# facebookresearch/SEAL

Measured on NVIDIA H100. Metric: queries/sec at beam=15, 1k queries, 10M-token index; rank-kernel HBM GB/s, higher is better.
Workload: dtype f32

## Files before the change

### include/sealdec.h

```cpp
#ifndef SEALDEC_H
#define SEALDEC_H
#include <stdint.h>
#include "sealfm.h"

#ifdef __cplusplus
extern "C" {
#endif


typedef struct {
    int32_t num_beams;
    int32_t pad_token_id;
    int32_t eos_token_id;
    int32_t stop_at_count;
    int32_t always_allow_eos;
    int32_t forced_bos_token_id;
    int32_t n_force_decoding_from;
    const int64_t* force_decoding_from;
    int32_t shift;
} sealdec_processor_cfg_t;

int sealdec_apply_index_mask_d(const sealfm_t* fm, sealfm_stream_t stream,
                               const sealdec_processor_cfg_t* cfg,
                               const int64_t* input_ids_d, int64_t R, int64_t t,
// ... 118 lines not shown
                           int64_t Q, int64_t S, const int64_t* dec_ids, const int32_t* row_query,
                           int64_t N, int64_t T, float temperature, float* out_logprob,
                           int64_t out_full_pos, float* out_full);

int sealdec_debug_step_logits(sealbart_t* model, const int64_t* input_ids, const int64_t* attention_mask,
                              int64_t Q, int64_t S, int32_t num_beams, const int64_t* decoder_input_ids,
                              int64_t t, float* out_logits);
int sealdec_debug_step_logits_ex(sealbart_t* model, const int64_t* input_ids, const int64_t* attention_mask,
                                 int64_t Q, int64_t S, int32_t num_beams, const int64_t* decoder_input_ids,
                                 int64_t t, const int32_t* ancestry, int64_t src_tokens_hint, float* out_logits);
int sealdec_debug_gemm(int mode, int64_t M, int32_t N, int32_t K, const float* A, const float* W,
                       const float* bias, float* C, int32_t gelu, int32_t iters, double* avg_us);
int sealdec_debug_gemm_ex(int mode, int64_t M, int32_t N, int32_t K, const float* A, const float* W,
                          const float* bias, float* C, int32_t gelu, int32_t iters, double* avg_us, int32_t band,
                          int32_t store);
int sealdec_debug_head(int64_t M, int32_t N, int32_t K, const float* A, const float* W, const float* bias,
                       const uint32_t* mask, int32_t eos, int32_t pad, float* C, float* stats, int32_t* fused);
int sealdec_debug_head_ex(int mode, int64_t M, int32_t N, int32_t K, const float* A, const float* W, const float* bias,
                          const uint32_t* mask, int32_t eos, int32_t pad, float* C, float* stats, int32_t* fused);
int sealdec_debug_select_step(const sealfm_t* fm, const sealdec_params_t* p, const sealdec_groups_t* groups, int64_t Q,
                              int32_t V, int32_t cur_len, int32_t logits_shared, int32_t logits_ignored,
                              const float* logits, const float* head_stats, const uint32_t* masks,
                              const uint32_t* occurring_mask, const float* beam_scores, const int32_t* tokens,
                              const int32_t* ancestry, const uint64_t* lo, const uint64_t* hi, const uint64_t* pw,
                              float* row_max, float* row_logsum, uint8_t* row_rule, float* cand_val, int32_t* cand_idx,
                              int32_t* cand_cnt, int32_t* lists, float* beam_scores_out, int32_t* tokens_out,
                              int32_t* ancestry_out, uint64_t* lo_out, uint64_t* hi_out, uint64_t* pw_out,
                              float* rec_score, int32_t* rec_len, int32_t* rec_tokens, uint8_t* rec_valid,
                              uint64_t* rec_lo, uint64_t* rec_hi, int32_t* error_flag);
int sealdec_debug_target_logprob(int64_t R, int32_t V, int64_t ld, const float* logits, const int64_t* targets,
                                 int64_t tgt_stride, float temperature, float* out, int64_t out_stride, float* full,
                                 int64_t full_ld);
typedef struct {
    int32_t kind, arch, d, heads;
    int64_t Q, S;
    int32_t B, pos, T, compact;
    const float* qkv; const float* q; const float* ckv;
    const float* kc; const float* vc; const int32_t* anc;
    const int32_t* src_mask; const int32_t* src_off;
    int64_t G; const int32_t* grp_query; const int32_t* grp_start;
    const float* rel_bias; int32_t num_buckets, max_distance;
    const float* split_part; int32_t split_ks; float split_unscale; const float* split_bias;
    int32_t out_split;
} sealdec_attn_case_t;
int sealdec_debug_attention(const sealdec_attn_case_t* c, float* out, void* split1, void* split2, void* split3,
                            int32_t* overflow, float* kc_out, float* vc_out, uint32_t* path);
int sealdec_debug_topk_threshold(int64_t R, int32_t V, int64_t ld, const float* logits, int32_t top_k, float* out_thr,
                                 float* out_max, float* out_logsum);
int sealdec_debug_topk_threshold_cluster(int64_t R, int32_t V, int64_t ld, const float* logits, int32_t top_k,
                                         float* out_thr, float* out_max, float* out_logsum);
int sealdec_debug_topk_rows(int64_t R, int32_t V, int32_t num_beams, int32_t per_row, int32_t iters, double* avg_us);
int sealdec_debug_gemm_trace(int enable, int64_t out20[20]);
int sealdec_debug_gemm_units(int64_t* out, int32_t n);
int64_t sealdec_last_launch_count(const sealbart_t* model);
int sealdec_profile_gemm(sealbart_t* model, int enable, double* total_us, int64_t* launches, double* flops);
int sealdec_last_phase_us(const sealbart_t* model, double out5[5]);

#ifdef __cplusplus
}
#endif
#endif
```

### seal_b200/_lib.py

```python
import ctypes as C
import os

_HERE = os.path.dirname(os.path.abspath(__file__))
LIB_PATH = os.path.join(_HERE, "libsealb200.so")

u64 = C.c_uint64
u32 = C.c_uint32
i32 = C.c_int
vp = C.c_void_p
cp = C.c_char_p


class SealB200Error(RuntimeError):
    def __init__(self, code, msg):
        super().__init__(f"[sealb200 {code}] {msg}")
        self.code = code


def _load():
    if not os.path.exists(LIB_PATH):
        raise ImportError(
            f"{LIB_PATH} not found: build it with `python -c 'import __graft_entry__ as g; g.build()'` "
            "or `make -C seal_b200/csrc`. seal_b200 has no CPU fallback.")
    return C.CDLL(LIB_PATH)
# ... 97 lines not shown
                ("B", C.c_int32), ("pos", C.c_int32), ("T", C.c_int32), ("compact", C.c_int32),
                ("qkv", vp), ("q", vp), ("ckv", vp), ("kc", vp), ("vc", vp), ("anc", vp),
                ("src_mask", vp), ("src_off", vp),
                ("G", C.c_int64), ("grp_query", vp), ("grp_start", vp),
                ("rel_bias", vp), ("num_buckets", C.c_int32), ("max_distance", C.c_int32),
                ("split_part", vp), ("split_ks", C.c_int32), ("split_unscale", C.c_float), ("split_bias", vp),
                ("out_split", C.c_int32)]


_DEC_SIGS = {
    "sealdec_apply_index_mask_d": (i32, [vp, vp, C.POINTER(ProcessorCfg), vp, C.c_int64, C.c_int64, vp, vp, vp,
                                         C.c_int64, C.c_int64]),
    "sealbart_create": (i32, [C.POINTER(BartConfig), i32, C.POINTER(vp)]),
    "sealbart_create_ex": (i32, [C.POINTER(BartConfig), C.POINTER(BartVariant), i32, C.POINTER(vp)]),
    "sealbart_free": (None, [vp]),
    "sealt5_create": (i32, [C.POINTER(T5Config), i32, C.POINTER(vp)]),
    "sealt5_relative_buckets": (i32, [C.c_int32, C.c_int32, C.c_int32, C.c_int32, vp]),
    "sealbart_set_tensor": (i32, [vp, cp, vp, u64]),
    "sealbart_finalize": (i32, [vp]),
    "sealbart_device_bytes": (u64, [vp]),
    "sealdec_hyps_per_query": (C.c_int64, [C.POINTER(DecParams)]),
    "sealdec_generate": (i32, [vp, vp, vp, C.POINTER(DecParams), vp, vp, C.c_int64, C.c_int64, vp, vp, vp, vp, vp, vp]),
    "sealdec_generate_d": (i32, [vp, vp, vp, C.POINTER(DecParams), vp, vp, C.c_int64, C.c_int64, vp, vp, vp, vp, vp,
                                 vp, vp, vp]),
    "sealdec_generate_dx": (i32, [vp, vp, vp, C.POINTER(DecParams), vp, vp, C.c_int64, C.c_int64, vp, vp, vp, vp, vp,
                                  vp, vp, vp, C.c_int64]),
    "sealdec_generate_ex": (i32, [vp, vp, vp, C.POINTER(DecParams), vp, vp, C.c_int64, C.c_int64, vp, vp, vp, vp, vp, vp,
                                  C.POINTER(GroupParams)]),
    "sealdec_generate_dx_ex": (i32, [vp, vp, vp, C.POINTER(DecParams), vp, vp, C.c_int64, C.c_int64, vp, vp, vp, vp, vp,
                                     vp, vp, vp, C.c_int64, C.POINTER(GroupParams)]),
    "sealbart_set_option": (i32, [vp, cp, C.c_int64]),
    "sealbart_get_stat": (C.c_int64, [vp, cp]),
    "sealdec_teacher_forced": (i32, [vp, vp, vp, C.c_int64, C.c_int64, vp, vp, C.c_int64, C.c_int64, C.c_float, vp,
                                     C.c_int64, vp]),
    "sealdec_debug_step_logits": (i32, [vp, vp, vp, C.c_int64, C.c_int64, C.c_int32, vp, C.c_int64, vp]),
    "sealdec_debug_step_logits_ex": (i32, [vp, vp, vp, C.c_int64, C.c_int64, C.c_int32, vp, C.c_int64, vp, C.c_int64,
                                           vp]),
    "sealdec_debug_gemm": (i32, [i32, C.c_int64, C.c_int32, C.c_int32, vp, vp, vp, vp, C.c_int32, C.c_int32,
                                 C.POINTER(C.c_double)]),
    "sealdec_debug_gemm_ex": (i32, [i32, C.c_int64, C.c_int32, C.c_int32, vp, vp, vp, vp, C.c_int32, C.c_int32,
                                    C.POINTER(C.c_double), C.c_int32, C.c_int32]),
    "sealdec_debug_head": (i32, [C.c_int64, C.c_int32, C.c_int32, vp, vp, vp, vp, C.c_int32, C.c_int32, vp, vp, vp]),
    "sealdec_debug_head_ex": (i32, [i32, C.c_int64, C.c_int32, C.c_int32, vp, vp, vp, vp, C.c_int32, C.c_int32, vp, vp, vp]),
    "sealdec_debug_select_step": (i32, [vp, C.POINTER(DecParams), C.POINTER(GroupParams), C.c_int64, C.c_int32, C.c_int32,
                                        C.c_int32, C.c_int32] + [vp] * 30),
    "sealdec_debug_target_logprob": (i32, [C.c_int64, C.c_int32, C.c_int64, vp, vp, C.c_int64, C.c_float, vp, C.c_int64,
                                           vp, C.c_int64]),
    "sealdec_debug_attention": (i32, [C.POINTER(AttnCase), vp, vp, vp, vp, vp, vp, vp, vp]),
    "sealdec_debug_topk_threshold": (i32, [C.c_int64, C.c_int32, C.c_int64, vp, C.c_int32, vp, vp, vp]),
    "sealdec_debug_topk_threshold_cluster": (i32, [C.c_int64, C.c_int32, C.c_int64, vp, C.c_int32, vp, vp, vp]),
    "sealdec_debug_topk_rows":(i32, [C.c_int64, C.c_int32, C.c_int32, C.c_int32, C.c_int32, C.POINTER(C.c_double)]),
    "sealdec_debug_gemm_trace": (i32, [i32, C.POINTER(C.c_int64)]),
    "sealdec_debug_gemm_units": (i32, [C.POINTER(C.c_int64), C.c_int32]),
    "sealev_first_stage": (i32, [C.c_int64, vp, vp, vp, vp, C.c_int64, vp, vp, vp, i32, i32, C.c_double, C.c_double, C.c_int64, vp, vp]),
    "sealev_score_docs": (i32, [C.c_int64, vp, vp, vp, vp, C.c_int64, C.c_int64, vp, vp, vp, C.c_int64, i32, i32, i32, i32,
                                C.c_double, C.c_double, vp, vp, vp, vp, vp, vp, C.c_int64]),
    "sealev_last_error": (C.c_char_p, []),
    "sealev_set_sum_mode": (None, [i32]),
    "sealev_key_scores": (i32, [C.c_int64, vp, vp, vp, vp, C.c_double, C.c_double, C.c_double, C.c_double, i32, vp]),
    "sealev_unigram_topk": (i32, [C.c_int64, C.c_int64, vp, C.c_int64, vp, vp, vp, vp]),
    "sealev_unigram_scores": (i32, [C.c_int64, vp, vp, vp, C.c_double, C.c_double, C.c_double, i32, vp]),
    "sealev_best_unigrams": (i32, [C.c_int64, vp, vp, vp, vp, vp, vp, vp, vp, C.c_int64]),
    "sealev_set_device_budget": (None, [u64]),
    "sealev_batch_first_stage": (i32, [vp, C.c_int64, vp, vp, vp, vp, vp, vp, vp, vp, i32, i32, C.c_double, C.c_double,
                                       C.c_int64, vp, vp, C.c_int64]),
    "sealev_batch_score_docs": (i32, [vp, C.c_int64, vp, vp, vp, vp, vp, vp, vp, vp, vp, vp, vp, vp, C.c_int64, i32, i32,
                                      i32, i32, C.c_double, C.c_double, vp, vp, C.c_int64, vp, vp, vp, vp, vp, vp,
                                      C.c_int64, vp]),
    "sealev_batch_phase_us": (None, [vp]),
    "sealdec_last_launch_count": (C.c_int64, [vp]),
    "sealdec_profile_gemm": (i32, [vp, i32, C.POINTER(C.c_double), C.POINTER(C.c_int64), C.POINTER(C.c_double)]),
    "sealdec_last_phase_us": (i32, [vp, C.POINTER(C.c_double)]),
}


def _bind(sigs):
    for name, (res, args) in sigs.items():
        fn = getattr(lib, name)
        fn.restype = res
        fn.argtypes = args


_bind(_FM_SIGS)
_bind(_DEC_SIGS)


def check(code):
    if code != 0:
        raise SealB200Error(code, lib.sealfm_last_error().decode(errors="replace"))


def fm_symbols():
    return list(_FM_SIGS)
```

### seal_b200/csrc/bart_kernels.cuh

```cuda
#pragma once
#include <cuda_bf16.h>
#include <cuda_fp16.h>
#include <cuda_runtime.h>
#include <cstdint>

#include "decode_types.cuh"
#include "launch.cuh"

namespace sealb200 {

__device__ __forceinline__ float warp_sum(float v) {
#pragma unroll
    for (int o = 16; o > 0; o >>= 1) v += __shfl_xor_sync(0xffffffffu, v, o);
    return v;
}
__device__ __forceinline__ float warp_max(float v) {
#pragma unroll
    for (int o = 16; o > 0; o >>= 1) v = fmaxf(v, __shfl_xor_sync(0xffffffffu, v, o));
    return v;
}

__device__ __forceinline__ void split1(float x, float& h, float& l) {
    h = __uint_as_float(__float_as_uint(x) & 0xFFFFE000u);
    l = x - h;
// ... 334 lines not shown
        if (rd * 4 < n_keys && s < n_keys) {
            const float p = expf(sc[rd] - mloc);
            lsum += p;
            const float4 v0 = vf[rd][0], v1 = vf[rd][1];
            a0.x = fmaf(p, v0.x, a0.x); a0.y = fmaf(p, v0.y, a0.y); a0.z = fmaf(p, v0.z, a0.z); a0.w = fmaf(p, v0.w, a0.w);
            a1.x = fmaf(p, v1.x, a1.x); a1.y = fmaf(p, v1.y, a1.y); a1.z = fmaf(p, v1.z, a1.z); a1.w = fmaf(p, v1.w, a1.w);
        }
    }
#pragma unroll
    for (int o = 8; o <= 16; o <<= 1) {
        lsum += __shfl_xor_sync(0xffffffffu, lsum, o);
        a0.x += __shfl_xor_sync(0xffffffffu, a0.x, o); a0.y += __shfl_xor_sync(0xffffffffu, a0.y, o);
        a0.z += __shfl_xor_sync(0xffffffffu, a0.z, o); a0.w += __shfl_xor_sync(0xffffffffu, a0.w, o);
        a1.x += __shfl_xor_sync(0xffffffffu, a1.x, o); a1.y += __shfl_xor_sync(0xffffffffu, a1.y, o);
        a1.z += __shfl_xor_sync(0xffffffffu, a1.z, o); a1.w += __shfl_xor_sync(0xffffffffu, a1.w, o);
    }
    const float inv = 1.0f / lsum;
    o0 = make_float4(a0.x * inv, a0.y * inv, a0.z * inv, a0.w * inv);
    o1 = make_float4(a1.x * inv, a1.y * inv, a1.z * inv, a1.w * inv);
}

template <int ROUNDS, class SO>
__global__ void __launch_bounds__(512, ROUNDS <= 3 ? 2 : 1) dec_self_attn_kernel(int64_t R, int d, int heads, int cur_pos, int T,
                                                               const float* __restrict__ qkv, float* kc, float* vc,
                                                               const int32_t* __restrict__ anc,
                                                               float* __restrict__ out, SO so, int row_mul, int bcast) {
    const int64_t r = blockIdx.x;
    const int64_t pr = r * row_mul;
    const int lane = threadIdx.x & 31, warp = threadIdx.x >> 5;
    const int g = lane >> 3, i8 = (lane & 7) * 8;
    const int n_keys = cur_pos + 1;
    const int32_t* arow = anc + pr * T;
    for (int h = warp; h < heads; h += blockDim.x >> 5) {
        const int col = h * kHeadDim + i8;
        const float* qp = qkv + r * 3 * d + col;
        float4 o0, o1;
        self_attend_head<ROUNDS>(qp, kc, vc, arow, R, d, col, cur_pos, n_keys, g, o0, o1);
        if (g == 0) {
            const int64_t idx = r * d + col;
            if (out) { *reinterpret_cast<float4*>(out + idx) = o0; *reinterpret_cast<float4*>(out + idx + 4) = o1; }
            store_split4(so, idx, o0); store_split4(so, idx + 4, o1);
            const float* kcur = qp + d; const float* vcur = qp + 2 * d;
            const float4 k0 = __ldg(reinterpret_cast<const float4*>(kcur)), k1 = __ldg(reinterpret_cast<const float4*>(kcur + 4));
            const float4 v0 = __ldg(reinterpret_cast<const float4*>(vcur)), v1 = __ldg(reinterpret_cast<const float4*>(vcur + 4));
            for (int b2 = 0; b2 < bcast; ++b2) {
                float* kd = kc + ((int64_t)cur_pos * R + pr + b2) * d + col; float* vd = vc + ((int64_t)cur_pos * R + pr + b2) * d + col;
                *reinterpret_cast<float4*>(kd) = k0; *reinterpret_cast<float4*>(kd + 4) = k1;
                *reinterpret_cast<float4*>(vd) = v0; *reinterpret_cast<float4*>(vd + 4) = v1;
            }
        }
    }
}

__host__ __device__ inline size_t self_attn_query_smem(int P, int B) { return (size_t)2 * P * B * kHeadDim * 4 + (size_t)2 * P * 32 * 4 + 128 * 4; }

template <class SO>
__global__ void __launch_bounds__(1024) dec_self_attn_query_kernel(int64_t R, int B, int d, int cur_pos, int T,
                                                                  const float* __restrict__ qkv, float* kc, float* vc,
                                                                  const int32_t* __restrict__ anc,
                                                                  float* __restrict__ out, SO so, SplitSrc qsrc) {
    extern __shared__ __align__(16) unsigned char sa_smem[];
    const int P = cur_pos + 1;
    float* Ks = reinterpret_cast<float*>(sa_smem);
    float* Vs = Ks + (size_t)P * B * kHeadDim;
    int32_t* row_of = reinterpret_cast<int32_t*>(Vs + (size_t)P * B * kHeadDim);
    int32_t* slot_of = row_of + P * 32;
    int32_t* ucount = slot_of + P * 32;
    const int64_t qi = blockIdx.x;
    const int col = blockIdx.y * kHeadDim;
    const int64_t r0 = qi * B;
    const int lane = threadIdx.x & 31, warp = threadIdx.x >> 5;
    for (int s = warp; s < P; s += B) {
        const bool act = lane < B;
        const unsigned amask = __ballot_sync(0xffffffffu, act);
        if (act) {
            const int a = (s == cur_pos) ? lane : anc[(r0 + lane) * T + s];
            const unsigned same = __match_any_sync(amask, a);
            const int leader = __ffs(same) - 1;
            const unsigned leaders = __ballot_sync(amask, leader == lane);
            slot_of[s * 32 + lane] = __popc(leaders & ((1u << leader) - 1u));
            if (leader == lane) row_of[s * 32 + __popc(leaders & ((1u << lane) - 1u))] = a;
            if (lane == 0) ucount[s] = __popc(leaders);
        }
    }
    __syncthreads();
    const int per_pos = B * (kHeadDim / 4);
    for (int e = threadIdx.x; e < P * per_pos; e += blockDim.x) {
        const int s = e / per_pos, rem = e - s * per_pos, slot = rem / (kHeadDim / 4), i4 = rem - slot * (kHeadDim / 4);
        if (slot >= ucount[s]) continue;
        const int a = row_of[s * 32 + slot];
        float4 kk, vv;
        if (s == cur_pos) {
            const int64_t qoff = (r0 + a) * 3 * d + col + 4 * i4;
            kk = load_split4(qkv, qsrc, qoff + d, d + col + 4 * i4); vv = load_split4(qkv, qsrc, qoff + 2 * d, 2 * d + col + 4 * i4);
            const int64_t off = ((int64_t)cur_pos * R + r0 + a) * d + col + 4 * i4;
            *reinterpret_cast<float4*>(kc + off) = kk; *reinterpret_cast<float4*>(vc + off) = vv;
        } else {
            const int64_t off = ((int64_t)s * R + a) * d + col + 4 * i4;
            kk = *reinterpret_cast<const float4*>(kc + off); vv = *reinterpret_cast<const float4*>(vc + off);
        }
        *reinterpret_cast<float4*>(Ks + ((size_t)s * B + slot) * kHeadDim + 4 * i4) = kk;
        *reinterpret_cast<float4*>(Vs + ((size_t)s * B + slot) * kHeadDim + 4 * i4) = vv;
    }
    __syncthreads();
    if (warp < B) {
        const int64_t r = r0 + warp;
        const float2 q2 = load_split2(qkv, qsrc, r * 3 * d + col + 2 * lane, col + 2 * lane);
        float m = -INFINITY, l = 0.f, ax = 0.f, ay = 0.f;
        for (int s = 0; s < P; ++s) {
            const int slot = slot_of[s * 32 + warp];
            const float2 k2 = *reinterpret_cast<const float2*>(Ks + ((size_t)s * B + slot) * kHeadDim + 2 * lane);
            const float sc = warp_sum(q2.x * k2.x + q2.y * k2.y) * 0.125f;
            const float mn = fmaxf(m, sc);
            const float corr = (m == -INFINITY) ? 0.f : expf(m - mn);
            const float p = expf(sc - mn);
            const float2 v2 = *reinterpret_cast<const float2*>(Vs + ((size_t)s * B + slot) * kHeadDim + 2 * lane);
            l = l * corr + p;
            ax = fmaf(p, v2.x, ax * corr); ay = fmaf(p, v2.y, ay * corr);
            m = mn;
        }
        store_attn(make_float2(ax / l, ay / l), r * d + col + 2 * lane, out, so);
    }
}

struct AncestryKV {
    const float* kc; const float* vc; const int32_t* arow; const float* kcur; const float* vcur;
    int64_t R; int d; int col; int cur_pos;
    __device__ __forceinline__ bool valid(int) const { return true; }
    __device__ __forceinline__ const float* k(int s) const { return s == cur_pos ? kcur : kc + ((int64_t)s * R + arow[s]) * d + col; }
    __device__ __forceinline__ const float* v(int s) const { return s == cur_pos ? vcur : vc + ((int64_t)s * R + arow[s]) * d + col; }
};

template <class SO>
__global__ void __launch_bounds__(512) dec_self_attn_long_kernel(int64_t R, int d, int heads, int cur_pos, int T,
                                                                 const float* __restrict__ qkv, float* kc, float* vc,
                                                                 const int32_t* __restrict__ anc,
                                                                 float* __restrict__ out, SO so) {
    __shared__ __align__(16) float q_s[16][kHeadDim];
    const int64_t r = blockIdx.x;
    const int lane = threadIdx.x & 31, warp = threadIdx.x >> 5;
    const int32_t* arow = anc + r * T;
    for (int h = warp; h < heads; h += blockDim.x >> 5) {
        const int col = h * kHeadDim;
        const float* qp = qkv + r * 3 * d + col;
        AncestryKV kv{kc, vc, arow, qp + d, qp + 2 * d, R, d, col, cur_pos};
        const float2 o = warp_attend(qp, cur_pos + 1, kv, q_s[warp]);
        store_attn(o, r * d + col + 2 * lane, out, so);
        const float2 k2 = *reinterpret_cast<const float2*>(qp + d + 2 * lane);
        const float2 v2 = *reinterpret_cast<const float2*>(qp + 2 * d + 2 * lane);
        *reinterpret_cast<float2*>(kc + ((int64_t)cur_pos * R + r) * d + col + 2 * lane) = k2;
        *reinterpret_cast<float2*>(vc + ((int64_t)cur_pos * R + r) * d + col + 2 * lane) = v2;
    }
}

struct GroupAddr {
    const float* q; int64_t q_stride;
    const float* k; const float* v; int64_t kv_stride;
    const int32_t* mask;
};

template <int NW, int MAXP, class SO>
__device__ __forceinline__ void grouped_attention(const GroupAddr& g, int rows, int n_keys, int head_off, int64_t out_base,
                                                  int64_t out_stride, float* __restrict__ out, const SO& so) {
    __shared__ float Kt[kHeadDim][33];
    __shared__ __align__(16) float Vs[32][kHeadDim];
    __shared__ __align__(16) float q_s[NW * MAXP][kHeadDim];
    __shared__ int32_t valid_s[32];
    const int lane = threadIdx.x & 31, warp = threadIdx.x >> 5;
    for (int rbase = 0; rbase < rows; rbase += NW * MAXP) {
        float m[MAXP], l[MAXP], ax[MAXP], ay[MAXP];
        bool has[MAXP];
#pragma unroll
        for (int p = 0; p < MAXP; ++p) {
            const int r = rbase + p * NW + warp;
// ... 194 lines not shown
```

### seal_b200/csrc/decode_model.hpp

```cpp
#pragma once
#include "../../include/sealdec.h"
#include "common.cuh"
#include "decode_types.cuh"

#include <cuda.h>
#include <cuda_bf16.h>
#include <cuda_fp16.h>
#include <cuda_runtime.h>

#include <cstdint>
#include <map>
#include <set>
#include <string>
#include <utility>
#include <vector>

#pragma GCC visibility push(hidden)

namespace sealb200 {

struct Lin {
    float* w = nullptr; float* b = nullptr; int out = 0, in = 0;
    float* w_hi = nullptr; float* w_lo = nullptr;
    __half* w_h1 = nullptr; __half* w_h2 = nullptr;
// ... 84 lines not shown
    int graph_policy = -1;
    int last_used_graph = 0;
    bool tf32_ready = false;
    int64_t overflow_fallbacks = 0;
    cudaStream_t stream = nullptr;
    int query_slices = -1;
    cudaStream_t slice_stream = nullptr;
    cudaEvent_t slice_fork = nullptr, slice_join = nullptr;
    Buf a_hi1, a_lo1, splitk1, st_wide1;
    Buf effn2, dffn2;
    ~sealbart() { for (void* p : allocs) cudaFree(p); for (void* p : split_allocs) cudaFree(p); }
};

namespace sealb200 {

enum GemmMode : int { kGemmTf32 = 2, kGemmFp16 = 3, kGemmFp16Cluster = 5, kGemmBf16 = 6 };
inline bool is_3xfp16(int64_t mode) { return mode == kGemmFp16 || mode == kGemmFp16Cluster; }
inline bool head_stats_mode(int mode) { return mode == kGemmFp16 || mode == kGemmBf16; }
inline bool bf16_weights(const sealbart* m) { return m->cfg.gemm_mode == kGemmBf16; }

constexpr int64_t kAddLnRowMax = 2048;

struct Act {
    float* x = nullptr; float* hi = nullptr; float* lo = nullptr;
    __half* h1 = nullptr; __half* h2 = nullptr;
    __nv_bfloat16* b1 = nullptr; __nv_bfloat16* b2 = nullptr; __nv_bfloat16* b3 = nullptr;
};

struct Ctx { sealbart* m; cudaStream_t s; SplitSrc pending{}; HeadEpi head{}; bool head_fused = false; int slice = 0; };

struct Dims {
    int64_t Q, S, R; int B, T, d, f, V, ld, W;
    int64_t G = 0; const int32_t* grp_query = nullptr; const int32_t* grp_start = nullptr;
    int64_t q0 = 0, r0 = 0, Qb = 0, Rb = 0;
};

template <typename Fn> void for_each_lin(sealbart* m, Fn&& fn) {
    for (auto& L : m->enc) { fn(L.qkv); fn(L.o); fn(L.fc1); fn(L.fc2); }
    for (auto& L : m->dec) { fn(L.qkv); fn(L.o); fn(L.cq); fn(L.ckv); fn(L.co); fn(L.fc1); fn(L.fc2); }
    fn(m->head);
}

void make_lin(sealbart* m, Lin& l, int out, int in);
void upload(void* dst, bool bf16, const float* host, uint64_t n, float scale = 1.f);
void check_model(const sealbart* m);
int require_device();
void ensure_workspace(sealbart* m, const Dims& D);
int32_t t5_bucket(int32_t rel, bool bidirectional, int num_buckets, int max_distance);

void gemm(Ctx& cx, int64_t M, int N, int K, const Act& A, int lda, Lin& l, const Act& C, int ldc, int act, int64_t defer_rows = 0);
void derive_lin(sealbart* m, Lin& l, unsigned int* d_max);
void ensure_tf32_splits(sealbart* m);
void check_gemm_mode(int mode);

void encoder_forward(Ctx& cx, const Dims& D, const int64_t* ids_d, const int64_t* mask_d, int64_t src_tokens_hint = -1,
                     int32_t* hint_err = nullptr);
void decoder_step(Ctx& cx, const Dims& D, const int32_t* tokens, int cur_len, const int32_t* anc, bool want_logits,
                  cudaEvent_t ev_layers_done, bool compact = false, const HeadEpi& head = HeadEpi{});

void drop_graphs(sealbart* m);

}

#pragma GCC visibility pop
```

### seal_b200/csrc/forward.cu

```cuda
#include "decode_model.hpp"
#include "bart_kernels.cuh"
#include "preln_kernels.cuh"
#include "t5_kernels.cuh"

#include <cuda_runtime.h>

#include <algorithm>
#include <cmath>
#include <cstdlib>
#include <type_traits>
#include <vector>

namespace {

SplitSrc take_pending(Ctx& cx) {
    const SplitSrc ps = cx.pending;
    cx.pending = SplitSrc{};
    return ps;
}

SplitOut split_of(const Act& a, int* overflow) {
    SplitOut so;
    if (a.hi) { so.a = a.hi; so.b = a.lo; so.kind = 1; }
    else if (a.h1) { so.a = a.h1; so.b = a.h2; so.kind = 2; so.overflow = overflow; }
// ... 68 lines not shown
    int64_t run = part[t];
    for (int64_t q = q0; q < q1; ++q) {
        src_off[q] = (int32_t)run;
        int len = 0;
        for (int s2 = 0; s2 < S; ++s2) len += mask[q * S + s2] != 0;
        run += len;
    }
    if (t == 0) src_off[Q] = (int32_t)info[0];
}

__global__ void prep_enc_packed_kernel(int64_t n, int S, const int64_t* __restrict__ ids, const int32_t* __restrict__ src_off,
                                       int32_t* __restrict__ tok, int32_t* __restrict__ pos) {
    const int64_t i = blockIdx.x * (int64_t)blockDim.x + threadIdx.x;
    if (i >= n) return;
    const int64_t q = i / S; const int s2 = (int)(i % S);
    if (s2 < src_off[q + 1] - src_off[q]) { const int64_t dst = src_off[q] + s2; tok[dst] = (int32_t)ids[i]; pos[dst] = s2; }
}

void t5_rms(Ctx& cx, int64_t rows, int d, const int32_t* tok, int64_t tok_stride, const Act& x, const float* b, const float* w,
            float out_scale) {
    const SplitSrc ps = take_pending(cx);
    const bool wide = d > 4 * 128 * kT5RmsVec;
    with_split(cx.m, x, [&](auto so) {
        using SO = decltype(so);
        launch_k(wide ? t5_rms_row_kernel<kT5RmsVecWide, SO> : t5_rms_row_kernel<kT5RmsVec, SO>, (unsigned)rows, 128, 0, cx.s, rows, d, tok, tok_stride,
                 embed_table<SO>(cx.m), x.x, b, ps, w, cx.m->t5.layer_norm_epsilon, out_scale, so);
    });
    cx.m->launches++;
    cx.m->last_paths |= wide ? kPathT5RmsWide : kPathT5Rms;
}

void t5_ffn(Ctx& cx, int64_t rows, int d, int f, const Act& x, Lin& fc1, Lin& fc2, const Act& ffn, float* ffn2, const Act& tmp) {
    sealbart* m = cx.m;
    if (m->t5.ffn_kind == 1) {
        gemm(cx, rows, 2 * f, d, x, d, fc1, Act{ffn2}, 2 * f, kActNone);
        const int blocks = (int)std::max<int64_t>(1, std::min<int64_t>((rows * (f / 4) + 255) / 256, (int64_t)sm_count() * 8));
        with_split(m, ffn, [&](auto so) { launch_k(t5_gate_kernel<decltype(so)>, (unsigned)blocks, 256, 0, cx.s, rows, f, (const float*)ffn2, so); });
        m->launches++; m->last_paths |= kPathT5Gate;
    } else
        gemm(cx, rows, f, d, x, d, fc1, ffn, f, kActRelu);
    gemm(cx, rows, d, f, ffn, f, fc2, tmp, d, kActNone, INT64_MAX);
}

struct Acts { Act x, qkv, attn, tmp, cq, ffn; float* ffn2 = nullptr; };

struct DecStep : Acts {
    int64_t R = 0, Rc = 0, Tk = 0, ckv_q0 = 0; int row_mul = 1, pos = 0; bool compact = false;
    const int32_t* tokens = nullptr; const int32_t* anc = nullptr; const int32_t* m32 = nullptr; const int32_t* soff_x = nullptr;
};


bool use_self_attn_query(int pos, int B, bool compact, bool ragged) {
    static const bool sa_query = [] { const char* e = std::getenv("SEALB200_SELF_ATTN_QUERY"); return !e || std::atoi(e) != 0; }();
    const size_t saq_smem = self_attn_query_smem(pos + 1, B);
    return sa_query && !compact && !ragged && pos >= 1 && B >= 2 && B <= 32 && pos + 1 <= 128 && saq_smem <= 112 * 1024;
}

bool use_cross_attn_small(int64_t S) { return S <= kXKeys; }

struct SelfAttnArgs {
    int64_t Q, R, Rc; int B, d, heads, pos, T, row_mul;
    const float* qkv; float* kc; float* vc; const int32_t* anc; float* out;
};

template <class SO>
uint32_t launch_bart_self_attn(cudaStream_t s, const SelfAttnArgs& a, bool use_saq, const SO& so, const SplitSrc& qkv_src) {
    const unsigned sa_threads = 32 * std::min(a.heads, 16);
    if (use_saq) {
        static size_t saq_set = 0;
        const size_t saq_smem = self_attn_query_smem(a.pos + 1, a.B);
        if (saq_smem > saq_set) { CUDA_CHECK(cudaFuncSetAttribute(dec_self_attn_query_kernel<SO>, cudaFuncAttributeMaxDynamicSharedMemorySize, 112 * 1024)); saq_set = 112 * 1024; }
        launch_k(dec_self_attn_query_kernel<SO>, dim3((unsigned)a.Q, a.heads), 32 * a.B, saq_smem, s, a.Rc, a.B, a.d, a.pos, a.T, a.qkv, a.kc, a.vc, a.anc,
                 a.out, so, qkv_src);
        return kPathSelfQuery;
    }
    if (a.pos + 1 <= 12) {
        launch_k(dec_self_attn_kernel<3, SO>, (unsigned)a.R, sa_threads, 0, s, a.Rc, a.d, a.heads, a.pos, a.T, a.qkv, a.kc, a.vc, a.anc, a.out, so, a.row_mul, a.row_mul);
        return kPathSelfRounds3;
    }
    if (a.pos + 1 <= 32) {
        launch_k(dec_self_attn_kernel<8, SO>, (unsigned)a.R, sa_threads, 0, s, a.Rc, a.d, a.heads, a.pos, a.T, a.qkv, a.kc, a.vc, a.anc, a.out, so, a.row_mul, a.row_mul);
        return kPathSelfRounds8;
    }
    launch_k(dec_self_attn_long_kernel<SO>, (unsigned)a.R, sa_threads, 0, s, a.Rc, a.d, a.heads, a.pos, a.T, a.qkv, a.kc, a.vc, a.anc, a.out, so);
    return kPathSelfLong;
}

template <class SO>
uint32_t launch_t5_dec_self_attn(cudaStream_t s, const SelfAttnArgs& a, const RelBias& rb, const SO& so) {
    launch_k(t5_dec_self_attn_kernel<SO>, (unsigned)a.R, 32 * std::min(a.heads, 16), 0, s, a.Rc, a.d, a.heads, a.pos, a.T, a.qkv, a.kc, a.vc,
             a.anc, rb, so, a.row_mul, a.row_mul);
    return kPathT5DecAttn;
}

struct CrossAttnArgs {
    int64_t groups; int d, heads, beams, S;
    const float* q; const float* ckv; const int32_t* mask; const int32_t* grp_query; const int32_t* grp_start; float* out;
    const int32_t* src_off;
};

template <class SO>
uint32_t launch_cross_attn(cudaStream_t s, const CrossAttnArgs& a, const SO& so, const SplitSrc& q_src) {
    if (use_cross_attn_small(a.S)) {
        launch_k(cross_attn_small_kernel<SO>, dim3((unsigned)a.groups, a.heads), 128, 0, s, a.groups, a.d, a.heads, a.beams, a.S, a.q,
                 a.ckv, a.mask, a.grp_query, a.grp_start, a.out, so, a.src_off, q_src);
        return kPathCrossSmall;
    }
    launch_k(cross_attn_kernel<SO>, dim3((unsigned)a.groups, a.heads), kGAttnWarps * 32, 0, s, a.groups, a.d, a.heads, a.beams, a.S, a.q,
             a.ckv, a.mask, a.grp_query, a.grp_start, a.out, so, a.src_off);
    return kPathCrossGrouped;
}

template <class SO>
uint32_t launch_enc_self_attn(cudaStream_t s, int64_t Q, int d, int heads, int S, const float* qkv, const int32_t* mask,
                              const RelBias* rb, float* out, const SO& so, const int32_t* src_off) {
    if (rb) {
        launch_k(t5_enc_self_attn_kernel<kGAttnWarps, kGAttnPasses, SO>, dim3((unsigned)Q, heads), kGAttnWarps * 32, 0, s, Q, d, S, qkv, mask, *rb,
                 so, src_off);
        return kPathT5EncAttn;
    }
    launch_k(enc_self_attn_kernel<SO>, dim3((unsigned)Q, heads), kGAttnWarps * 32, 0, s, Q, d, heads, S, qkv, mask, out, so, src_off);
    return 0;
}

void cross_attention(Ctx& cx, const Dims& D, const DecStep& S, int l, int64_t defer_rows) {
    sealbart* m = cx.m;
// ... 347 lines not shown
            else up(d_mask, c->src_mask, (size_t)Q * c->S * 4);
        }
        const size_t cache_bytes = self ? (size_t)c->T * Rc * d * 4 : 0;
        if (self) {
            up(d_kc, c->kc, cache_bytes); up(d_vc, c->vc, cache_bytes); up(d_anc, c->anc, (size_t)Rc * c->T * 4);
            const size_t at_pos = (size_t)c->pos * Rc * d * 4, pos_bytes = (size_t)Rc * d * 4;
            CUDA_CHECK(cudaMemset(d_kc.as<char>() + at_pos, 0xFF, pos_bytes)); CUDA_CHECK(cudaMemset(d_vc.as<char>() + at_pos, 0xFF, pos_bytes));
        }
        if (cross && c->G) { up(d_gq, c->grp_query, (size_t)c->G * 4); up(d_gs, c->grp_start, (size_t)(c->G + 1) * 4); }
        RelBias rb{};
        if (t5_bias) {
            const int off = enc ? kT5MaxSource - 1 : kMaxLen - 1;
            std::vector<int32_t> bkt(enc ? 2 * kT5MaxSource - 1 : kMaxLen);
            for (int i = 0; i < (int)bkt.size(); ++i) bkt[i] = t5_bucket(i - off, enc, c->num_buckets, c->max_distance);
            up(d_bkt, bkt.data(), bkt.size() * 4); up(d_rel, c->rel_bias, (size_t)c->num_buckets * heads * 4);
            rb = RelBias{d_rel.as<float>(), d_bkt.as<int32_t>(), off, heads};
        }
        const size_t out_n = (size_t)rows * d, piece = c->out_split == 1 ? 4 : 2;
        nan(d_out, out_n * 4);
        if (c->out_split) { nan(d_s1, out_n * piece); nan(d_s2, out_n * piece); }
        if (c->out_split == 3) nan(d_s3, out_n * piece);
        d_ovf.ensure(4); CUDA_CHECK(cudaMemset(d_ovf.p, 0, 4));
        SplitSrc src{};
        if (c->split_ks > 1) src = SplitSrc{d_part.as<float>(), c->split_ks, (int64_t)rows * cols, d_pb.as<float>(), c->split_unscale};

        const float* in = d_in.as<float>();
        const int32_t* mask = c->src_off ? nullptr : d_mask.as<int32_t>();
        const int32_t* soff = c->src_off ? d_off.as<int32_t>() : nullptr;
        auto run = [&](auto so) -> uint32_t {
            if (enc) return launch_enc_self_attn(nullptr, Q, d, heads, (int)c->S, in, mask, t5 ? &rb : nullptr, d_out.as<float>(), so, soff);
            if (self) {
                const SelfAttnArgs a{Q, rows, Rc, c->B, d, heads, c->pos, c->T, c->compact ? c->B : 1, in, d_kc.as<float>(), d_vc.as<float>(),
                                     d_anc.as<int32_t>(), d_out.as<float>()};
                return t5 ? launch_t5_dec_self_attn(nullptr, a, rb, so) : launch_bart_self_attn(nullptr, a, use_saq, so, src);
            }
            const CrossAttnArgs a{c->G ? c->G : Q, d, heads, c->compact ? 1 : c->B, (int)c->S, in, d_ckv.as<float>(), mask,
                                  c->G ? d_gq.as<int32_t>() : nullptr, c->G ? d_gs.as<int32_t>() : nullptr, d_out.as<float>(), soff};
            return launch_cross_attn(nullptr, a, so, src);
        };
        uint32_t bit;
        if (c->out_split == 3) bit = run(SplitBf16{d_s1.as<__nv_bfloat16>(), d_s2.as<__nv_bfloat16>(), d_s3.as<__nv_bfloat16>()});
        else bit = run(SplitOut{d_s1.p, d_s2.p, c->out_split, c->out_split == 2 ? d_ovf.as<int>() : nullptr});
        CUDA_CHECK(cudaDeviceSynchronize());
        auto down = [&](void* h, const Buf& b, size_t bytes) { CUDA_CHECK(cudaMemcpy(h, b.p, bytes, cudaMemcpyDeviceToHost)); };
        down(out, d_out, out_n * 4);
        if (c->out_split) { down(split1, d_s1, out_n * piece); down(split2, d_s2, out_n * piece); }
        if (c->out_split == 3) down(split3, d_s3, out_n * piece);
        if (overflow) down(overflow, d_ovf, 4);
        if (self) { down(kc_out, d_kc, cache_bytes); down(vc_out, d_vc, cache_bytes); }
        *path = bit;
    });
}

}
```

### seal_b200/csrc/gemm.cu

```cuda
#include "decode_model.hpp"
#include "wgmma_gemm.cuh"

#include <cuda_runtime.h>

#include <algorithm>
#include <cmath>
#include <cstdlib>
#include <cstring>
#include <iterator>
#include <type_traits>
#include <vector>

namespace {

typedef CUresult (*EncodeTiledFn)(CUtensorMap*, CUtensorMapDataType, cuuint32_t, void*, const cuuint64_t*, const cuuint64_t*,
                                  const cuuint32_t*, const cuuint32_t*, CUtensorMapInterleave, CUtensorMapSwizzle,
                                  CUtensorMapL2promotion, CUtensorMapFloatOOBfill);
EncodeTiledFn encode_tiled() {
    static EncodeTiledFn fn = nullptr;
    if (!fn) {
        void* p = nullptr;
        cudaDriverEntryPointQueryResult q;
        CUDA_CHECK(cudaGetDriverEntryPoint("cuTensorMapEncodeTiled", &p, cudaEnableDefault, &q));
        if (!p || q != cudaDriverEntryPointSuccess) throw ApiError(SEALFM_ECUDA, "cuTensorMapEncodeTiled unavailable");
// ... 206 lines not shown
}

void split_lin_half(sealbart* m, Lin& l, unsigned int* d_max) {
    const uint64_t n = (uint64_t)l.out * l.in;
    CUDA_CHECK(cudaMemset(d_max, 0, 4));
    absmax_kernel<<<sm_count() * 4, 256>>>((int64_t)n, l.w, d_max);
    unsigned int bits = 0; CUDA_CHECK(cudaMemcpy(&bits, d_max, 4, cudaMemcpyDeviceToHost));
    float mx; std::memcpy(&mx, &bits, 4);
    int sexp = 0;
    if (mx > 0.f) { int e; std::frexp(mx, &e); sexp = 14 - e; }
    l.w_unscale = std::ldexp(1.0f, -sexp);
    CUDA_CHECK(cudaMalloc(&l.w_h1, n * 2)); m->split_allocs.push_back(l.w_h1);
    CUDA_CHECK(cudaMalloc(&l.w_h2, n * 2)); m->split_allocs.push_back(l.w_h2);
    m->weight_bytes += 2 * n * 2;
    split_half_kernel<<<sm_count() * 8, 256>>>((int64_t)n, l.w, std::ldexp(1.0f, sexp), l.w_h1, l.w_h2, m->err.as<int>() + 1);
    CUDA_CHECK(cudaGetLastError());
    l.maps_ready = false;
}

}

namespace sealb200 {

void gemm(Ctx& cx, int64_t M, int N, int K, const Act& A, int lda, Lin& l, const Act& C, int ldc, int act, int64_t defer_rows) {
    sealbart* m = cx.m;
    if (!m->profile_gemm || M == 0) { gemm_impl(cx, M, N, K, A, lda, l, C, ldc, act, defer_rows); return; }
    cudaEvent_t a, b;
    CUDA_CHECK(cudaEventCreate(&a)); CUDA_CHECK(cudaEventCreate(&b));
    CUDA_CHECK(cudaEventRecord(a, cx.s));
    gemm_impl(cx, M, N, K, A, lda, l, C, ldc, act, defer_rows);
    CUDA_CHECK(cudaEventRecord(b, cx.s));
    m->gemm_events.emplace_back(a, b);
    m->gemm_flops += 2.0 * (double)M * N * K;
}

void derive_lin(sealbart* m, Lin& l, unsigned int* d_max) {
    if (m->cfg.gemm_mode == kGemmTf32) split_lin_tf32(m, l);
    else if (is_3xfp16(m->cfg.gemm_mode)) split_lin_half(m, l, d_max);
}

void ensure_tf32_splits(sealbart* m) {
    if (m->tf32_ready) return;
    CUDA_CHECK(cudaSetDevice(m->device));
    for_each_lin(m, [&](Lin& l) { split_lin_tf32(m, l); });
    CUDA_CHECK(cudaDeviceSynchronize());
    m->tf32_ready = true;
}

void check_gemm_mode(int mode) {
    if (mode != kGemmTf32 && !is_3xfp16(mode) && mode != kGemmBf16)
        throw ApiError(SEALFM_EINVAL, "gemm_mode must be 3 (3xFP16, one CTA per tile, default), 5 (3xFP16 on 2-CTA clusters), 2 (3xTF32) "
                                      "or 6 (3xBF16, bf16 weights)");
}

}


extern "C" {

int sealdec_debug_gemm_trace(int enable, int64_t out20[20]) {
    return guarded([&] {
        if (out20) {
            CUDA_CHECK(cudaDeviceSynchronize());
            long long h[20];
            CUDA_CHECK(cudaMemcpyFromSymbol(h, g_gemm_trace, sizeof(h)));
            for (int i = 0; i < 20; ++i) out20[i] = h[i];
        }
        const int on = enable ? 1 : 0;
        CUDA_CHECK(cudaMemcpyToSymbol(g_gemm_trace_on, &on, sizeof(int)));
    });
}

int sealdec_debug_gemm_units(int64_t* out, int32_t n) {
    return guarded([&] {
        if (!out || n < 0 || n > 4 * kTraceUnits) throw ApiError(SEALFM_EINVAL, "out is null or n is outside [0, 4 * 256]");
#ifndef SEAL_GEMM_UNIT_TRACE
        throw ApiError(SEALFM_EINVAL, "built without the per-unit GEMM timeline (make GEMM_UNIT_TRACE=1)");
#endif
        CUDA_CHECK(cudaDeviceSynchronize());
        std::vector<long long> h(4 * kTraceUnits);
        CUDA_CHECK(cudaMemcpyFromSymbol(h.data(), g_gemm_units, h.size() * sizeof(long long)));
        for (int i = 0; i < n; ++i) out[i] = h[i];
        std::fill(h.begin(), h.end(), 0ll);
        CUDA_CHECK(cudaMemcpyToSymbol(g_gemm_units, h.data(), h.size() * sizeof(long long)));
    });
}

int sealdec_profile_gemm(sealbart_t* m, int enable, double* total_us, int64_t* launches, double* flops) {
    return guarded([&] {
        if (!m) throw ApiError(SEALFM_EINVAL, "null model");
        CUDA_CHECK(cudaSetDevice(m->device));
        if (total_us && launches && flops) {
            CUDA_CHECK(cudaDeviceSynchronize());
            double us = 0;
            for (auto& e : m->gemm_events) { float ms = 0; CUDA_CHECK(cudaEventElapsedTime(&ms, e.first, e.second)); us += (double)ms * 1e3; }
            *total_us = us; *launches = (int64_t)m->gemm_events.size(); *flops = m->gemm_flops;
        }
        for (auto& e : m->gemm_events) { cudaEventDestroy(e.first); cudaEventDestroy(e.second); }
        m->gemm_events.clear(); m->gemm_flops = 0;
        m->profile_gemm = enable != 0;
    });
}

}

namespace {
// ... 94 lines not shown
```

Baseline: 2714.

## Restructure self-attention query kernel to fixed 256 threads with chunked KV staging

The decoder self-attention query kernel now runs with a fixed 256-thread block and stages K/V rows through a small shared-memory window of at most 32 rows, instead of loading every position's unique ancestor rows at once with up to 1024 threads and up to 112KB of shared memory. Per-position unique ancestor rows are compacted with a prefix sum, and the kernel walks them in chunks that fit the window, with each warp handling two beams. This lowers per-block shared memory and register footprint so several blocks can be resident per SM and overlap with other kernels. In exchange it adds a syncthreads pair per chunk, caps P*B at 224, and adds a debug function that reports kernel resource footprints.

```diff
diff --git a/include/sealdec.h b/include/sealdec.h
--- a/include/sealdec.h
+++ b/include/sealdec.h
@@ -194,6 +194,7 @@
 int sealdec_debug_topk_rows(int64_t R, int32_t V, int32_t num_beams, int32_t per_row, int32_t iters, double* avg_us);
 int sealdec_debug_gemm_trace(int enable, int64_t out20[20]);
 int sealdec_debug_gemm_units(int64_t* out, int32_t n);
+int sealdec_debug_self_attn_fit(int32_t out_split, int64_t out[12]);
 int64_t sealdec_last_launch_count(const sealbart_t* model);
 int sealdec_profile_gemm(sealbart_t* model, int enable, double* total_us, int64_t* launches, double* flops);
 int sealdec_last_phase_us(const sealbart_t* model, double out5[5]);
diff --git a/seal_b200/_lib.py b/seal_b200/_lib.py
--- a/seal_b200/_lib.py
+++ b/seal_b200/_lib.py
@@ -173,6 +173,7 @@
     "sealdec_debug_topk_rows":(i32, [C.c_int64, C.c_int32, C.c_int32, C.c_int32, C.c_int32, C.POINTER(C.c_double)]),
     "sealdec_debug_gemm_trace": (i32, [i32, C.POINTER(C.c_int64)]),
     "sealdec_debug_gemm_units": (i32, [C.POINTER(C.c_int64), C.c_int32]),
+    "sealdec_debug_self_attn_fit": (i32, [i32, C.POINTER(C.c_int64)]),
     "sealev_first_stage": (i32, [C.c_int64, vp, vp, vp, vp, C.c_int64, vp, vp, vp, i32, i32, C.c_double, C.c_double, C.c_int64, vp, vp]),
     "sealev_score_docs": (i32, [C.c_int64, vp, vp, vp, vp, C.c_int64, C.c_int64, vp, vp, vp, C.c_int64, i32, i32, i32, i32,
                                 C.c_double, C.c_double, vp, vp, vp, vp, vp, vp, C.c_int64]),
diff --git a/seal_b200/csrc/bart_kernels.cuh b/seal_b200/csrc/bart_kernels.cuh
--- a/seal_b200/csrc/bart_kernels.cuh
+++ b/seal_b200/csrc/bart_kernels.cuh
@@ -410,25 +410,44 @@
     }
 }
 
-__host__ __device__ inline size_t self_attn_query_smem(int P, int B) { return (size_t)2 * P * B * kHeadDim * 4 + (size_t)2 * P * 32 * 4 + 128 * 4; }
+constexpr int kSaqThreads = 256, kSaqRows = 32, kSaqMaxPB = 224;
+__host__ __device__ inline int self_attn_query_rows(int P, int B) { return P * B < kSaqRows ? P * B : kSaqRows; }
+__host__ __device__ inline size_t self_attn_query_smem(int P, int B) { return (size_t)2 * self_attn_query_rows(P, B) * kHeadDim * 4; }
 
 template <class SO>
-__global__ void __launch_bounds__(1024) dec_self_attn_query_kernel(int64_t R, int B, int d, int cur_pos, int T,
-                                                                  const float* __restrict__ qkv, float* kc, float* vc,
-                                                                  const int32_t* __restrict__ anc,
-                                                                  float* __restrict__ out, SO so, SplitSrc qsrc) {
+__global__ void __launch_bounds__(kSaqThreads, 4)  dec_self_attn_query_kernel(int64_t R, int B, int d, int cur_pos, int T,
+                                                                           const float* __restrict__ qkv, float* kc, float* vc,
+                                                                           const int32_t* __restrict__ anc,
+                                                                           float* __restrict__ out, SO so, SplitSrc qsrc) {
+    constexpr int NW = kSaqThreads / 32, NB = 2;
+    constexpr int F4 = kHeadDim / 4;
+    constexpr int PER = (kSaqRows * F4 + kSaqThreads - 1) / kSaqThreads;
+    constexpr int PER0 = (32 * F4 + kSaqThreads - 1) / kSaqThreads;
     extern __shared__ __align__(16) unsigned char sa_smem[];
+    __shared__ int64_t row_s[kSaqMaxPB];
+    __shared__ int32_t base_s[kMaxLen + 1];
+    __shared__ int32_t anc_s[kSaqMaxPB];
+    __shared__ uint8_t slot_s[kSaqMaxPB];
+    __shared__ uint8_t cnt_s[kMaxLen];
     const int P = cur_pos + 1;
+    const int cap = self_attn_query_rows(P, B);
     float* Ks = reinterpret_cast<float*>(sa_smem);
-    float* Vs = Ks + (size_t)P * B * kHeadDim;
-    int32_t* row_of = reinterpret_cast<int32_t*>(Vs + (size_t)P * B * kHeadDim);
-    int32_t* slot_of = row_of + P * 32;
-    int32_t* ucount = slot_of + P * 32;
+    float* Vs = Ks + (size_t)cap * kHeadDim;
     const int64_t qi = blockIdx.x;
     const int col = blockIdx.y * kHeadDim;
     const int64_t r0 = qi * B;
     const int lane = threadIdx.x & 31, warp = threadIdx.x >> 5;
-    for (int s = warp; s < P; s += B) {
+    float4 kq[PER0], vq[PER0];
+#pragma unroll
+    for (int i = 0; i < PER0; ++i) {
+        const int e = threadIdx.x + i * kSaqThreads;
+        if (e < B * F4) {
+            const int b = e / F4, i4 = e % F4;
+            const int64_t qoff = (r0 + b) * 3 * d + col + 4 * i4;
+            kq[i] = load_split4(qkv, qsrc, qoff + d, d + col + 4 * i4); vq[i] = load_split4(qkv, qsrc, qoff + 2 * d, 2 * d + col + 4 * i4);
+        }
+    }
+    for (int s = warp; s < P; s += NW) {
         const bool act = lane < B;
         const unsigned amask = __ballot_sync(0xffffffffu, act);
         if (act) {
@@ -436,48 +455,104 @@
             const unsigned same = __match_any_sync(amask, a);
             const int leader = __ffs(same) - 1;
             const unsigned leaders = __ballot_sync(amask, leader == lane);
-            slot_of[s * 32 + lane] = __popc(leaders & ((1u << leader) - 1u));
-            if (leader == lane) row_of[s * 32 + __popc(leaders & ((1u << lane) - 1u))] = a;
-            if (lane == 0) ucount[s] = __popc(leaders);
+            const int slot = __popc(leaders & ((1u << leader) - 1u));
+            slot_s[s * B + lane] = (uint8_t)slot;
+            if (leader == lane) anc_s[s * B + slot] = a;
+            if (lane == 0) cnt_s[s] = (uint8_t)__popc(leaders);
+        }
+    }
+#pragma unroll
+    for (int i = 0; i < PER0; ++i) {
+        const int e = threadIdx.x + i * kSaqThreads;
+        if (e < B * F4) {
+            const int b = e / F4, i4 = e % F4;
+            const int64_t off = ((int64_t)cur_pos * R + r0 + b) * d + col + 4 * i4;
+            *reinterpret_cast<float4*>(kc + off) = kq[i]; *reinterpret_cast<float4*>(vc + off) = vq[i];
         }
     }
     __syncthreads();
-    const int per_pos = B * (kHeadDim / 4);
-    for (int e = threadIdx.x; e < P * per_pos; e += blockDim.x) {
-        const int s = e / per_pos, rem = e - s * per_pos, slot = rem / (kHeadDim / 4), i4 = rem - slot * (kHeadDim / 4);
-        if (slot >= ucount[s]) continue;
-        const int a = row_of[s * 32 + slot];
-        float4 kk, vv;
-        if (s == cur_pos) {
-            const int64_t qoff = (r0 + a) * 3 * d + col + 4 * i4;
-            kk = load_split4(qkv, qsrc, qoff + d, d + col + 4 * i4); vv = load_split4(qkv, qsrc, qoff + 2 * d, 2 * d + col + 4 * i4);
-            const int64_t off = ((int64_t)cur_pos * R + r0 + a) * d + col + 4 * i4;
-            *reinterpret_cast<float4*>(kc + off) = kk; *reinterpret_cast<float4*>(vc + off) = vv;
-        } else {
-            const int64_t off = ((int64_t)s * R + a) * d + col + 4 * i4;
-            kk = *reinterpret_cast<const float4*>(kc + off); vv = *reinterpret_cast<const float4*>(vc + off);
-        }
-        *reinterpret_cast<float4*>(Ks + ((size_t)s * B + slot) * kHeadDim + 4 * i4) = kk;
-        *reinterpret_cast<float4*>(Vs + ((size_t)s * B + slot) * kHeadDim + 4 * i4) = vv;
+    if (warp == 0) {
+        int c[kMaxLen / 32], sum = 0;
+#pragma unroll
+        for (int i = 0; i < kMaxLen / 32; ++i) { const int s = 4 * lane + i; c[i] = s < P ? cnt_s[s] : 0; sum += c[i]; }
+        int incl = sum;
+#pragma unroll
+        for (int o = 1; o < 32; o <<= 1) { const int y = __shfl_up_sync(0xffffffffu, incl, o); if (lane >= o) incl += y; }
+        int run = incl - sum;
+#pragma unroll
+        for (int i = 0; i < kMaxLen / 32; ++i) { const int s = 4 * lane + i; if (s < P) base_s[s] = run; run += c[i]; }
+        if (lane == 31) base_s[P] = incl;
     }
     __syncthreads();
-    if (warp < B) {
-        const int64_t r = r0 + warp;
-        const float2 q2 = load_split2(qkv, qsrc, r * 3 * d + col + 2 * lane, col + 2 * lane);
-        float m = -INFINITY, l = 0.f, ax = 0.f, ay = 0.f;
-        for (int s = 0; s < P; ++s) {
-            const int slot = slot_of[s * 32 + warp];
-            const float2 k2 = *reinterpret_cast<const float2*>(Ks + ((size_t)s * B + slot) * kHeadDim + 2 * lane);
-            const float sc = warp_sum(q2.x * k2.x + q2.y * k2.y) * 0.125f;
-            const float mn = fmaxf(m, sc);
-            const float corr = (m == -INFINITY) ? 0.f : expf(m - mn);
-            const float p = expf(sc - mn);
-            const float2 v2 = *reinterpret_cast<const float2*>(Vs + ((size_t)s * B + slot) * kHeadDim + 2 * lane);
-            l = l * corr + p;
-            ax = fmaf(p, v2.x, ax * corr); ay = fmaf(p, v2.y, ay * corr);
-            m = mn;
-        }
-        store_attn(make_float2(ax / l, ay / l), r * d + col + 2 * lane, out, so);
+    if ((int)threadIdx.x < P * B) {
+        const int s = threadIdx.x / B, k = threadIdx.x - s * B;
+        if (k < cnt_s[s]) row_s[base_s[s] + k] = (int64_t)s * R + (s == cur_pos ? r0 : 0) + anc_s[threadIdx.x];
+    }
+    __syncthreads();
+    for (int b0 = 0; b0 < B; b0 += NW * NB) {
+    float2 q2[NB];
+    float m[NB], l[NB], ax[NB], ay[NB];
+#pragma unroll
+    for (int j = 0; j < NB; ++j) {
+        const int b = b0 + warp + NW * j;
+        q2[j] = make_float2(0.f, 0.f); m[j] = -INFINITY; l[j] = 0.f; ax[j] = 0.f; ay[j] = 0.f;
+        if (b < B) q2[j] = load_split2(qkv, qsrc, (r0 + b) * 3 * d + col + 2 * lane, col + 2 * lane);
+    }
+    for (int sa = 0; sa < P;) {
+        const int g0 = base_s[sa];
+        int sb = sa;
+        for (;;) {
+            const int s = sb + 1 + lane;
+            const unsigned fit = __ballot_sync(0xffffffffu, s <= P && base_s[s] - g0 <= cap);
+            sb += __popc(fit);
+            if (fit != 0xffffffffu) break;
+        }
+        const int n4 = (base_s[sb] - g0) * F4;
+        float4 kk[PER], vv[PER];
+#pragma unroll
+        for (int i = 0; i < PER; ++i) {
+            const int e = threadIdx.x + i * kSaqThreads;
+            if (e < n4) {
+                const int64_t off = row_s[g0 + e / F4] * d + col + 4 * (e % F4);
+                kk[i] = *reinterpret_cast<const float4*>(kc + off); vv[i] = *reinterpret_cast<const float4*>(vc + off);
+            }
+        }
+#pragma unroll
+        for (int i = 0; i < PER; ++i) {
+            const int e = threadIdx.x + i * kSaqThreads;
+            if (e < n4) {
+                *reinterpret_cast<float4*>(Ks + (size_t)e * 4) = kk[i];
+                *reinterpret_cast<float4*>(Vs + (size_t)e * 4) = vv[i];
+            }
+        }
+        __syncthreads();
+        for (int s = sa; s < sb; ++s) {
+            const int rb = base_s[s] - g0;
+#pragma unroll
+            for (int j = 0; j < NB; ++j) {
+                const int b = b0 + warp + NW * j;
+                if (b < B) {
+                    const size_t row = (size_t)(rb + slot_s[s * B + b]) * kHeadDim;
+                    const float2 k2 = *reinterpret_cast<const float2*>(Ks + row + 2 * lane);
+                    const float sc = warp_sum(q2[j].x * k2.x + q2[j].y * k2.y) * 0.125f;
+                    const float mn = fmaxf(m[j], sc);
+                    const float corr = (m[j] == -INFINITY) ? 0.f : expf(m[j] - mn);
+                    const float p = expf(sc - mn);
+                    const float2 v2 = *reinterpret_cast<const float2*>(Vs + row + 2 * lane);
+                    l[j] = l[j] * corr + p;
+                    ax[j] = fmaf(p, v2.x, ax[j] * corr); ay[j] = fmaf(p, v2.y, ay[j] * corr);
+                    m[j] = mn;
+                }
+            }
+        }
+        __syncthreads();
+        sa = sb;
+    }
+#pragma unroll
+    for (int j = 0; j < NB; ++j) {
+        const int b = b0 + warp + NW * j;
+        if (b < B) store_attn(make_float2(ax[j] / l[j], ay[j] / l[j]), (r0 + b) * d + col + 2 * lane, out, so);
+    }
     }
 }
 
diff --git a/seal_b200/csrc/decode_model.hpp b/seal_b200/csrc/decode_model.hpp
--- a/seal_b200/csrc/decode_model.hpp
+++ b/seal_b200/csrc/decode_model.hpp
@@ -160,6 +160,8 @@
 void derive_lin(sealbart* m, Lin& l, unsigned int* d_max);
 void ensure_tf32_splits(sealbart* m);
 void check_gemm_mode(int mode);
+struct GemmFootprint { int threads, regs_per_thread; size_t dyn_smem; };
+GemmFootprint gemm_footprint();
 
 void encoder_forward(Ctx& cx, const Dims& D, const int64_t* ids_d, const int64_t* mask_d, int64_t src_tokens_hint = -1,
                      int32_t* hint_err = nullptr);
diff --git a/seal_b200/csrc/forward.cu b/seal_b200/csrc/forward.cu
--- a/seal_b200/csrc/forward.cu
+++ b/seal_b200/csrc/forward.cu
@@ -144,8 +144,9 @@
 
 bool use_self_attn_query(int pos, int B, bool compact, bool ragged) {
     static const bool sa_query = [] { const char* e = std::getenv("SEALB200_SELF_ATTN_QUERY"); return !e || std::atoi(e) != 0; }();
-    const size_t saq_smem = self_attn_query_smem(pos + 1, B);
-    return sa_query && !compact && !ragged && pos >= 1 && B >= 2 && B <= 32 && pos + 1 <= 128 && saq_smem <= 112 * 1024;
+    const int P = pos + 1;
+    const size_t all_rows = (size_t)2 * P * B * kHeadDim * 4 + (size_t)2 * P * 32 * 4 + 128 * 4;
+    return sa_query && !compact && !ragged && pos >= 1 && B >= 2 && B <= 32 && P <= 128 && P * B <= kSaqMaxPB && all_rows <= 112 * 1024;
 }
 
 bool use_cross_attn_small(int64_t S) { return S <= kXKeys; }
@@ -159,11 +160,8 @@
 uint32_t launch_bart_self_attn(cudaStream_t s, const SelfAttnArgs& a, bool use_saq, const SO& so, const SplitSrc& qkv_src) {
     const unsigned sa_threads = 32 * std::min(a.heads, 16);
     if (use_saq) {
-        static size_t saq_set = 0;
-        const size_t saq_smem = self_attn_query_smem(a.pos + 1, a.B);
-        if (saq_smem > saq_set) { CUDA_CHECK(cudaFuncSetAttribute(dec_self_attn_query_kernel<SO>, cudaFuncAttributeMaxDynamicSharedMemorySize, 112 * 1024)); saq_set = 112 * 1024; }
-        launch_k(dec_self_attn_query_kernel<SO>, dim3((unsigned)a.Q, a.heads), 32 * a.B, saq_smem, s, a.Rc, a.B, a.d, a.pos, a.T, a.qkv, a.kc, a.vc, a.anc,
-                 a.out, so, qkv_src);
+        launch_k(dec_self_attn_query_kernel<SO>, dim3((unsigned)a.Q, a.heads), kSaqThreads, self_attn_query_smem(a.pos + 1, a.B), s, a.Rc, a.B,
+                 a.d, a.pos, a.T, a.qkv, a.kc, a.vc, a.anc, a.out, so, qkv_src);
         return kPathSelfQuery;
     }
     if (a.pos + 1 <= 12) {
@@ -617,4 +615,27 @@
     });
 }
 
-}
+int sealdec_debug_self_attn_fit(int32_t out_split, int64_t out[12]) {
+    return guarded([&] {
+        if (!out || out_split < 0 || out_split > 3) throw ApiError(SEALFM_EINVAL, "out is null or out_split is outside 0..3");
+        require_device();
+        cudaFuncAttributes fa{};
+        if (out_split == 3) CUDA_CHECK(cudaFuncGetAttributes(&fa, dec_self_attn_query_kernel<SplitBf16>));
+        else CUDA_CHECK(cudaFuncGetAttributes(&fa, dec_self_attn_query_kernel<SplitOut>));
+        size_t dyn = 0;
+        for (int pos = 0; pos < kMaxLen; ++pos)
+            for (int B = 1; B <= 32; ++B)
+                if (use_self_attn_query(pos, B, false, false)) dyn = std::max(dyn, self_attn_query_smem(pos + 1, B));
+        const GemmFootprint g = gemm_footprint();
+        int dev = 0, sm_regs = 0, sm_smem = 0, reserved = 0;
+        CUDA_CHECK(cudaGetDevice(&dev));
+        CUDA_CHECK(cudaDeviceGetAttribute(&sm_regs, cudaDevAttrMaxRegistersPerMultiprocessor, dev));
+        CUDA_CHECK(cudaDeviceGetAttribute(&sm_smem, cudaDevAttrMaxSharedMemoryPerMultiprocessor, dev));
+        CUDA_CHECK(cudaDeviceGetAttribute(&reserved, cudaDevAttrReservedSharedMemoryPerBlock, dev));
+        const int64_t v[12] = {fa.numRegs, (int64_t)fa.sharedSizeBytes, (int64_t)dyn, fa.maxThreadsPerBlock, kSaqThreads,
+                               (int64_t)fa.localSizeBytes, g.threads, g.regs_per_thread, (int64_t)g.dyn_smem, sm_regs, sm_smem, reserved};
+        std::copy(v, v + 12, out);
+    });
+}
+
+}
diff --git a/seal_b200/csrc/gemm.cu b/seal_b200/csrc/gemm.cu
--- a/seal_b200/csrc/gemm.cu
+++ b/seal_b200/csrc/gemm.cu
@@ -282,6 +282,8 @@
         throw ApiError(SEALFM_EINVAL, "gemm_mode must be 3 (3xFP16, one CTA per tile, default), 5 (3xFP16 on 2-CTA clusters), 2 (3xTF32) "
                                       "or 6 (3xBF16, bf16 weights)");
 }
+
+GemmFootprint gemm_footprint() { return GemmFootprint{GTHREADS, G_REGS, (size_t)G_SMEM}; }
 
 }
 
```

After: 2758, median of 6. +1.6%, better.
